# hilo-mpc/hilo-mpc

Hardware: AMD Instinct MI355X
Metric: MPC steps/sec (batched instances, whole node) at fixed (nx,nu,N) (higher is better)
Workload: dtype f64

## Files before the change

hilo_mpc_amd/csrc/hilo_nmpc_track.h:

```cpp
#pragma once
#include "hilo_ocp.h"

namespace hilo {

template <class M, bool BIG_ = false, bool SYM_ = true>
struct NmpcTrack {
  using Model = M;
  static constexpr bool SYM = SYM_ && ModelSym<M>::value && !model_has_ext<M>::value;
  static constexpr int NX = M::NX, NU = M::NU, NZ = NX + NU, NPAR = M::NP + M::NU, NSD = 0;
  static constexpr bool FIX_X0 = true;
  static constexpr bool BIG = BIG_;
  static constexpr int NC = 0, NXV = NX, NX0 = NX, NU0 = NU;
  static constexpr bool COOP = model_has_ext<M>::value;
  static constexpr bool QUAD_COST = true;
  static constexpr int O_WZ = 0, O_ZREF = O_WZ + NZ * NZ, O_WN = O_ZREF + NZ, O_XREFN = O_WN + NX * NX,
                       O_WDU = O_XREFN + NX, O_HASDU = O_WDU + NU * NU, O_SZ = O_HASDU + 1, O_SDU = O_SZ + NZ * NZ;
  static constexpr bool SYMTAB = O_SDU + NU * NU <= OCP_NCOST;
  static constexpr int O_END = SYMTAB ? O_SDU + NU * NU : O_SZ;
  static constexpr int NCOST = O_END;

  template <class T, class E>
  __device__ __forceinline__ static void dyn(const OcpConst& pc, const double* par, const double*, int, const T* x,
                                             const T* u, T* xn, const E& ext) {
    T xp[NX], up[NU > 0 ? NU : 1], xo[NX];
#pragma unroll
    for (int i = 0; i < NX; ++i) xp[i] = x[i] * pc.sz[i];
#pragma unroll
    for (int i = 0; i < NU; ++i) up[i] = u[i] * pc.sz[NX + i];
    model_step<M>(pc.order, pc.nsub, xp, up, par, pc.dt, xo, ext);
#pragma unroll
    for (int i = 0; i < NX; ++i) xn[i] = xo[i] * rcp_fast(pc.sz[i]);
  }

  static constexpr bool PLANT = !COOP;
  __device__ __forceinline__ static void plant(const OcpConst& pc, const double* par, const double* x, const double* u, double* xn) {
    if constexpr (PLANT) {
      double xv[NX], uv[NU > 0 ? NU : 1], pv[M::NP > 0 ? M::NP : 1], xo[NX];
#pragma unroll
      for (int i = 0; i < NX; ++i) xv[i] = x[i];
#pragma unroll
      for (int i = 0; i < NU; ++i) uv[i] = u[i];
#pragma unroll
      for (int i = 0; i < M::NP; ++i) pv[i] = par[i];
      model_step<M>(pc.order, pc.nsub, xv, uv, pv, pc.dt, xo);
#pragma unroll
      for (int i = 0; i < NX; ++i) xn[i] = xo[i];
    }
  }

  template <class T>
  __device__ __forceinline__ static T stage_cost(const OcpConst& pc, const double* par, const double*, int k,
                                                 const T* x, const T* u) {
    T z[NZ];
#pragma unroll
    for (int i = 0; i < NX; ++i) z[i] = x[i] - pc.cost[O_ZREF + i];
#pragma unroll
    for (int i = 0; i < NU; ++i) z[NX + i] = u[i] - pc.cost[O_ZREF + NX + i];
    T acc = T(0.0);
#pragma unroll
    for (int i0 = 0; i0 < NZ; i0 += 2) {
      double w[2][NZ];
#pragma unroll
      for (int a = 0; a < 2; ++a)
#pragma unroll
        for (int j = 0; j < NZ; ++j) w[a][j] = pc.cost[O_WZ + (i0 + a < NZ ? i0 + a : i0) * NZ + j];
      asm volatile("");
#pragma unroll
      for (int a = 0; a < 2; ++a) {
        if (i0 + a < NZ) {
          T s = T(0.0);
#pragma unroll
          for (int j = 0; j < NZ; ++j) s = s + w[a][j] * z[j];
          acc = acc + z[i0 + a] * s;
        }
      }
    }
    if (k == 0 && pc.cost[O_HASDU] != 0.0) {
      T d[NU > 0 ? NU : 1];
#pragma unroll
      for (int i = 0; i < NU; ++i) d[i] = u[i] - par[M::NP + i];
#pragma unroll
      for (int i = 0; i < NU; ++i) {
        T s = T(0.0);
#pragma unroll
        for (int j = 0; j < NU; ++j) s = s + pc.cost[O_WDU + i * NU + j] * d[j];
        acc = acc + d[i] * s;
      }
    }
    return acc;
  }

  __device__ __forceinline__ static double cost_grad(const OcpConst& pc, const double* par, const double*, int k, int i, const double* z) {
    double g = 0.0;
    {
      double wr[NZ], wc[NZ], zr[NZ];
#pragma unroll
      for (int j = 0; j < NZ; ++j) { wr[j] = pc.cost[O_WZ + i * NZ + j]; wc[j] = pc.cost[O_WZ + j * NZ + i]; zr[j] = pc.cost[O_ZREF + j]; }
      asm volatile("");
#pragma unroll
      for (int j = 0; j < NZ; ++j) g += (wr[j] + wc[j]) * (z[j] - zr[j]);
    }
    if (k == 0 && i >= NX && pc.cost[O_HASDU] != 0.0) {
#pragma unroll
      for (int j = 0; j < NU; ++j)
        g += (pc.cost[O_WDU + (i - NX) * NU + j] + pc.cost[O_WDU + j * NU + (i - NX)]) * (z[NX + j] - par[M::NP + j]);
    }
    return g;
  }
  __device__ __forceinline__ static double cost_hess(const OcpConst& pc, int k, int i, int j) {
    double h = pc.cost[O_WZ + i * NZ + j] + pc.cost[O_WZ + j * NZ + i];
    if (k == 0 && i >= NX && j >= NX && pc.cost[O_HASDU] != 0.0)
      h += pc.cost[O_WDU + (i - NX) * NU + (j - NX)] + pc.cost[O_WDU + (j - NX) * NU + (i - NX)];
    return h;
  }

  template <int CPL>
  __device__ __forceinline__ static void cost_cols(const OcpConst& pc, const double* par, int k, int c0, const double* z,
                                                   double* g, double (*ch)[CPL]) {
    static_assert(SYMTAB, "cost_cols needs the symmetrised tables");
    double S[NZ][CPL], zr[NZ], Sd[NU > 0 ? NU : 1][CPL], uo[NU > 0 ? NU : 1];
    int col[CPL], cu[CPL];
#pragma unroll
    for (int c = 0; c < CPL; ++c) {
      col[c] = c0 + c < NZ ? c0 + c : NZ - 1;
      cu[c] = col[c] >= NX ? col[c] - NX : 0;
    }
#pragma unroll
    for (int r = 0; r < NZ; ++r) {
      zr[r] = pc.cost[O_ZREF + r];
#pragma unroll
      for (int c = 0; c < CPL; ++c) S[r][c] = pc.cost[O_SZ + r * NZ + col[c]];
    }
#pragma unroll
    for (int a = 0; a < NU; ++a) {
      uo[a] = par[M::NP + a];
#pragma unroll
      for (int c = 0; c < CPL; ++c) Sd[a][c] = pc.cost[O_SDU + a * NU + cu[c]];
    }
    const bool du = k == 0 && pc.cost[O_HASDU] != 0.0;
#pragma unroll
    for (int c = 0; c < CPL; ++c) {
      double acc = 0.0;
#pragma unroll
      for (int r = 0; r < NZ; ++r) acc += S[r][c] * (z[r] - zr[r]);
      const bool duc = du && col[c] >= NX;
      double acd = acc;
#pragma unroll
      for (int a = 0; a < NU; ++a) acd += Sd[a][c] * (z[NX + a] - uo[a]);
      g[c] = duc ? acd : acc;
#pragma unroll
      for (int r = 0; r < NZ; ++r) {
        double h = S[r][c];
        if (r >= NX) h = duc ? h + Sd[r >= NX ? r - NX : 0][c] : h;
        ch[r][c] = (c0 + c < NZ && r >= c0 + c) ? h : 0.0;
      }
    }
  }

  __device__ __forceinline__ static double term_grad(const OcpConst& pc, int i, const double* x) {
    double g = 0.0;
#pragma unroll
    for (int j = 0; j < NX; ++j) g += (pc.cost[O_WN + i * NX + j] + pc.cost[O_WN + j * NX + i]) * (x[j] - pc.cost[O_XREFN + j]);
    return g;
  }
  __device__ __forceinline__ static double term_hess(const OcpConst& pc, int i, int j) {
    return pc.cost[O_WN + i * NX + j] + pc.cost[O_WN + j * NX + i];
  }

  template <class T>
  __device__ __forceinline__ static T term_cost(const OcpConst& pc, const double*, const double*, const T* x) {
    T z[NX];
#pragma unroll
    for (int i = 0; i < NX; ++i) z[i] = x[i] - pc.cost[O_XREFN + i];
    T acc = T(0.0);
// ... 24 lines not shown
```

hilo_mpc_amd/csrc/hilo_ocp.h:

```cpp
#pragma once
#include "hilo_colloc.h"
#include "hilo_common.h"
#include "hilo_models.h"

namespace hilo {

constexpr int OCP_MAXNX = 12, OCP_MAXNU = 8, OCP_MAXNZ = OCP_MAXNX + OCP_MAXNU;
constexpr int OCP_FILTER = 16;
constexpr int OCP_MAXNC = 16;
#ifndef HILO_OCP_TPB
#define HILO_OCP_TPB 64
#endif
#ifndef HILO_OCP_MINW
#define HILO_OCP_MINW 1
#endif
#ifdef HILO_OCP_INLINE_PHASES
#define OCP_PHASE __attribute__((always_inline))
#else
#define OCP_PHASE __attribute__((noinline))
#endif
constexpr int OCP_TPB = HILO_OCP_TPB;
constexpr int OCP_NCOST = 2 * OCP_MAXNZ * OCP_MAXNZ + 4 * OCP_MAXNZ + 64;

struct OcpConst {
// ... 379 lines not shown
    return (k > 0 && ((pc.k0_only_mask >> i) & 1u)) ? -INFINITY : pc.lbz[i];
  }
  __device__ static double ub_of(const OcpConst& pc, int k, int i) {
    if (k == 0 && (pc.flags & 2) && i < NX0) return pc.x0ub[i];
    return (k > 0 && ((pc.k0_only_mask >> i) & 1u)) ? INFINITY : pc.ubz[i];
  }

  __device__ __forceinline__ static void pair_of(int d, int n, int& i, int& j) {
    int r = d - n, ii = 0;
    for (int t = 0; t + 1 < n; ++t) {
      const int w = n - 1 - ii;
      const bool go = r >= w;
      r -= go ? w : 0;
      ii += go ? 1 : 0;
    }
    i = ii;
    j = ii + 1 + r;
  }
  __device__ static int dir_of(int i, int j, int n) { return n + i * (n - 1) - i * (i - 1) / 2 + (j - i - 1); }
  __device__ static bool pair_on(const OcpConst& pc, int d) {
    const int p = d - NZ;
    return p >= 256 || ((pc.pair_mask[p >> 6] >> (p & 63)) & 1ull) != 0ull;
  }
  __device__ static void build_dirs(const Lds l) {
    const OcpConst& pc = *(const OcpConst*)l.pc;
    if (threadIdx.x == 0) {
      int n = 0;
      for (int d = 0; d < NDIR; ++d)
        if (d < NZ || pair_on(pc, d)) l.dirs[1 + n++] = d;
      l.dirs[0] = n;
    }
    __syncthreads();
  }

  __device__ static const double* sd_of(const Lds l, int k) { return (const double*)(l.sd + (NSD > 0 ? k * NSD : 0)); }

  __device__ OCP_PHASE static FTheta eval_values_call(lds_double* lbase, double* ws, cvp Zp, ep cp, cdp sp, dp dstore, double extra) {
    lbase = uni(lbase); ws = uni(ws); Zp = uni(Zp); cp = uni(cp); sp = uni(sp); dstore = uni(dstore);
    const Lds l = carve(lbase, ws);
    const OcpConst& pc = *(const OcpConst*)l.pc;
    const int N = pc.N;
    double fpart = 0.0, tpart = 0.0;
    if constexpr (COOP) {
      const int lane = threadIdx.x;
      int gs = 64 / N;
      gs = gs < 1 ? 1 : gs;
      const int ng = 64 / gs, g = lane / gs, gl = lane - g * gs;
      const double* gp = (const double*)pc.ext;
      for (int r = 0; r * ng < N; ++r) {
        const int k = r * ng + g;
        const bool active = g < ng && k < N;
        const int kk = active ? k : N - 1;
        int nev = 0;
        const GpExt ext{gp, l.ext, gs, active ? gl : 0, active ? g * gs : lane, !active, (lds_cdouble*)(l.ext + NEXT_SCR),
                        pc.nsub == 1 ? l.gpc + kk * 24 : nullptr, &nev, false};
        double x[NX], u[NU > 0 ? NU : 1], xn[NX];
#pragma unroll
        for (int i = 0; i < NX; ++i) x[i] = Zp[kk * NZ + i];
#pragma unroll
        for (int i = 0; i < NU; ++i) u[i] = Zp[kk * NZ + NX + i];
        PB::dyn(pc, (const double*)l.par, sd_of(l, kk), kk, x, u, xn, ext);
        if (active && gl == 0) {
          fpart += PB::stage_cost(pc, (const double*)l.par, sd_of(l, k), k, x, u);
#pragma unroll
          for (int i = 0; i < NX; ++i) {
            const double ci = Zp[(k + 1) * NZ + i] - xn[i];
            cp[k * NX + i] = ci;
            tpart += fabs(ci);
          }
        }
      }
      if (lane == 63) {
        double x[NX];
#pragma unroll
        for (int i = 0; i < NX; ++i) x[i] = Zp[N * NZ + i];
        fpart += PB::term_cost(pc, (const double*)l.par, sd_of(l, N), x);
      }
    } else {
    if constexpr (XCW > 0) PB::template coll_pass<false>(pc, (const double*)l.par, (const double*)l.sd, Zp, l.lam, l.cnu, N, l.xc, l.prep, l.prepl,
                                                         uni((size_t)Zp != (size_t)l.Z));
#ifdef HILO_DBG_TWICE_VALS
    if constexpr (XCW > 0) PB::template coll_pass<false>(pc, (const double*)l.par, (const double*)l.sd, Zp, l.lam, l.cnu, N, l.xc, l.prep, l.prepl);
#endif
    OCP_FOR(k, (N) + 1) {
      double x[NX], u[NU > 0 ? NU : 1];
#pragma unroll
      for (int i = 0; i < NX; ++i) x[i] = Zp[k * NZ + i];
      if (k < N) {
        double xn[NX];
#pragma unroll
        for (int i = 0; i < NU; ++i) u[i] = Zp[k * NZ + NX + i];
        double dvf[NC > 0 ? NC : 1];
        if constexpr (XCW > 0) {
          fpart += PB::dyn_cost_xc(pc, (const double*)l.par, sd_of(l, k), k, x, u, xn, dvf, l.xc + (size_t)k * XCW);
        } else if constexpr (FUSED_CON) {
          static_assert(!FUSED_CON || FUSED, "fused rows need the fused cost");
          fpart += PB::dyn_cost_con(pc, (const double*)l.par, sd_of(l, k), k, x, u, xn, dvf, NoExt{});
        } else if constexpr (FUSED) {
          fpart += PB::dyn_cost(pc, (const double*)l.par, sd_of(l, k), k, x, u, xn, NoExt{});
        } else if constexpr (SYM) {
          using M = typename PB::Model;
          double xp[NX], up[NU > 0 ? NU : 1], X[4][NX], phi[NX];
#pragma unroll
          for (int i = 0; i < NX; ++i) xp[i] = x[i] * pc.sz[i];
#pragma unroll
          for (int i = 0; i < NU; ++i) up[i] = u[i] * pc.sz[NX + i];
          sym_points<M>(M::DISCRETE ? 1 : pc.order, pc.dt, xp, up, (const double*)l.par, X, phi);
          dp xs = l.Xs + (size_t)k * 4 * NX;
#pragma unroll
          for (int i = 0; i < 4; ++i)
#pragma unroll
            for (int q = 0; q < NX; ++q) xs[i * NX + q] = X[i][q];
#pragma unroll
          for (int i = 0; i < NX; ++i) xn[i] = phi[i] * rcp_fast(pc.sz[i]);
          fpart += PB::stage_cost(pc, (const double*)l.par, sd_of(l, k), k, x, u);
        } else {
          if constexpr (SYM_MHE) {
            FastD xf[NX], uf[NU > 0 ? NU : 1], xnf[NX];
#pragma unroll
            for (int i = 0; i < NX; ++i) xf[i] = FastD(x[i]);
#pragma unroll
            for (int i = 0; i < NU; ++i) uf[i] = FastD(u[i]);
            PB::dyn(pc, (const double*)l.par, sd_of(l, k), k, xf, uf, xnf, NoExt{});
#pragma unroll
            for (int i = 0; i < NX; ++i) xn[i] = xnf[i].v;
          } else {
            PB::dyn(pc, (const double*)l.par, sd_of(l, k), k, x, u, xn, NoExt{});
          }
          fpart += PB::stage_cost(pc, (const double*)l.par, sd_of(l, k), k, x, u);
        }
#pragma unroll
        for (int i = 0; i < NX; ++i) {
          const double ci = Zp[(k + 1) * NZ + i] - xn[i];
          cp[k * NX + i] = ci;
          tpart += fabs(ci);
        }
        if constexpr (NC > 0) {
          double dv[NC];
          if constexpr (FUSED_CON) {
#pragma unroll
            for (int m = 0; m < NC; ++m) dv[m] = dvf[m];
          } else PB::con(pc, (const double*)l.par, sd_of(l, k), k, x, u, xn, dv);
#pragma unroll
          for (int m = 0; m < NC; ++m) {
            if (row_on(pc, k, m)) {
              if (dstore) dstore[k * NC + m] = dv[m];
              if (sp) tpart += fabs(dv[m] - sp[k * NC + m]);
            }
          }
        }
      } else {
        fpart += PB::term_cost(pc, (const double*)l.par, sd_of(l, N), x);
      }
    }
    }
    if constexpr (OCP_TPB == 64) {
      double rv[3] = {fpart, tpart, extra};
      WaveReduceN<R_SUM, R_SUM, R_SUM>::run(rv);
      return FTheta{rv[0], rv[1], rv[2]};
    } else {
      const double fr = block_reduce<OpSum>(fpart, l.red);
      const double tr = block_reduce<OpSum>(tpart, l.red);
      return FTheta{fr, tr, block_reduce<OpSum>(extra, l.red)};
    }
  }

  __device__ __forceinline__ static FTheta eval_values(lds_double* lbase, double* ws, cvp Zp, ep cp, cdp sp = nullptr,
                                                      dp dstore = nullptr, double extra = 0.0) {
    const FTheta r = eval_values_call(lbase, ws, Zp, cp, sp, dstore, extra);
    return FTheta{uni(r.f), uni(r.theta), uni(r.x)};
  }

  template <bool TRIAL>
  __device__ __forceinline__ static double slots_log(const Lds l, cvp Zp, double alpha, int N) {
    constexpr int U = 2;
    const int SLT = (N + 1) * NZ;
    double part = 0.0;
    for (int base = 0; base < SLT; base += OCP_TPB * U) {
      double lbv[U], ubv[U], zv[U], dv[U];
      bool ok[U];
#pragma unroll
      for (int u = 0; u < U; ++u) {
        const int e0 = base + u * OCP_TPB + (int)threadIdx.x;
        ok[u] = e0 < SLT;
        const int e = ok[u] ? e0 : 0;
        lbv[u] = l.lbA[e]; ubv[u] = l.ubA[e]; zv[u] = Zp[e];
        dv[u] = TRIAL ? l.D[e] : 0.0;
      }
      double prod = 1.0;
      bool pos = true;
#pragma unroll
      for (int u = 0; u < U; ++u) {
        const double z = TRIAL ? zv[u] + alpha * dv[u] : zv[u];
        if constexpr (TRIAL) {
          if (ok[u]) l.Zt[base + u * OCP_TPB + (int)threadIdx.x] = z;
        }
        const bool hl = ok[u] && lbv[u] > -INFINITY, hu = ok[u] && ubv[u] < INFINITY;
        const double sl = hl ? z - lbv[u] : 1.0, su = hu ? ubv[u] - z : 1.0;
        prod *= sl * su;
        pos = pos && sl > 0.0 && su > 0.0;
      }
      const double r = -log(prod);
      part += pos ? r : __builtin_nan("");
    }
    return part;
  }
  __device__ static double barrier_logs(const Lds l, cvp Zp, cdp sp = nullptr) {
    const OcpConst& pc = *(const OcpConst*)l.pc;
    const int N = pc.N;
    double part = slots_log<false>(l, Zp, 0.0, N);
    if constexpr (NC > 0) {
      OCP_FOR(e, N * NC) {
        const int m = e % NC;
        if (!row_on(pc, e / NC, m)) continue;
        if (pc.dlb[m] > -INFINITY) part -= log(sp[e] - pc.dlb[m]);
        if (pc.dub[m] < INFINITY) part -= log(pc.dub[m] - sp[e]);
// ... 196 lines not shown
        if (d >= NX) pair_of(d, NX, di, dj);
        Jet2 x[NX];
#pragma unroll
        for (int i = 0; i < NX; ++i) x[i] = Jet2(l.Z[N * NZ + i], (i == di || i == dj) ? 1.0 : 0.0, 0.0);
        const Jet2 v = PB::term_cost(pc, (const double*)l.par, sd_of(l, N), x);
        qd_term(l, N)[d] = v.b;
        if (d < NX) l.grad[N * NZ + d] = v.a;
        if (d == 0) l.fk[N] = v.v;
      }
      }
    }
#ifdef HILO_DBG_TWICE_DIRS
    }
#endif
    __syncthreads();
    if constexpr (BIG) {
      constexpr int U = 4;
      const int total = N * NZ * NZ;
      for (int base = 0; base < total; base += OCP_TPB * U) {
        double qd[U], qa[U], qb[U];
        int kk[U], ii[U], jj[U];
        bool on[U], ok[U];
#pragma unroll
        for (int u = 0; u < U; ++u) {
          const int e0 = base + u * OCP_TPB + (int)threadIdx.x;
          ok[u] = e0 < total;
          const int e = ok[u] ? e0 : 0;
          const int k = e / (NZ * NZ), r = e - k * NZ * NZ, i = r / NZ, j = r - i * NZ;
          const int a = i < j ? i : j, b = i < j ? j : i;
          const int dd = i == j ? i : dir_of(a, b, NZ);
          cdp Q = l.Qd + k * NDIR;
          qd[u] = Q[dd]; qa[u] = Q[a]; qb[u] = Q[b];
          kk[u] = k; ii[u] = i; jj[u] = j;
          on[u] = i == j || COOP || pair_on(pc, dd);
        }
#pragma unroll
        for (int u = 0; u < U; ++u) {
          const int k = kk[u], i = ii[u], j = jj[u];
          double h = i == j ? qd[u] : (on[u] ? 0.5 * (qd[u] - qa[u] - qb[u]) : 0.0);
          if constexpr (PB::QUAD_COST) h += PB::cost_hess(pc, k, i, j);
          if (k == 0 && (((pinm >> i) | (pinm >> j)) & 1u)) h = 0.0;
          if (ok[u]) l.W[(k * NZ + i) * WP + j] = h;
        }
      }
    } else {
      OCP_FOR(e, N * NZ * NZ) {
        const int k = e / (NZ * NZ), r = e - k * NZ * NZ, i = r / NZ, j = r - i * NZ;
        cdp Q = l.Qd + k * NDIR;
        double h;
        if (i == j) h = Q[i];
        else {
          const int a = i < j ? i : j, b = i < j ? j : i, dd = dir_of(a, b, NZ);
          h = (COOP || pair_on(pc, dd)) ? 0.5 * (Q[dd] - Q[a] - Q[b]) : 0.0;
        }
        if constexpr (PB::QUAD_COST) h += PB::cost_hess(pc, k, i, j);
        if (k == 0 && (((pinm >> i) | (pinm >> j)) & 1u)) h = 0.0;
        l.W[(k * NZ + i) * WP + j] = h;
      }
    }
    if constexpr (PB::QUAD_COST) {
      OCP_FOR(e, N * NZ) {
        const int k = e / NZ, i = e - k * NZ;
        if (is_free(pc, k, i)) l.grad[e] = PB::cost_grad(pc, (const double*)l.par, sd_of(l, k), k, i, (const double*)(l.Z + k * NZ));
      }
      OCP_FOR(k, N) {
        double x[NX], u[NU > 0 ? NU : 1];
#pragma unroll
        for (int i = 0; i < NX; ++i) x[i] = l.Z[k * NZ + i];
#pragma unroll
        for (int i = 0; i < NU; ++i) u[i] = l.Z[k * NZ + NX + i];
        l.fk[k] = PB::stage_cost(pc, (const double*)l.par, sd_of(l, k), k, x, u);
      }
      __syncthreads();
    }
    double fpart = 0.0;
    OCP_FOR(k, (N) + 1) fpart += l.fk[k];
    OCP_FOR(a, NU) l.grad[N * NZ + NX + a] = 0.0;
    const double f = block_reduce<OpSum>(fpart, l.red);
    __syncthreads();
    return f;
  }


  template <class M>
  __device__ __forceinline__ static void sym_points(int order, double h, const double* x, const double* u, const double* par,
                                                    double (*X)[NX], double* phi) {
    constexpr bool DISC = M::DISCRETE;
    const double a10 = order >= 2 ? 0.5 : 0.0, a20 = order == 3 ? -1.0 : 0.0, a21 = order == 3 ? 2.0 : (order == 4 ? 0.5 : 0.0),
                 a32 = order == 4 ? 1.0 : 0.0;
    const double hb[4] = {DISC ? 1.0 : h * erk_b<0>(order), DISC ? 0.0 : h * erk_b<1>(order), DISC ? 0.0 : h * erk_b<2>(order),
                          DISC ? 0.0 : h * erk_b<3>(order)};
    FastD kk[4][NX], uf[NU > 0 ? NU : 1];
#pragma unroll
    for (int i = 0; i < NU; ++i) uf[i] = FastD(u[i]);
#pragma unroll
    for (int i = 0; i < 4; ++i) {
      FastD Xf[NX];
#pragma unroll
      for (int s = 0; s < NX; ++s) {
        double acc = x[s];
        if (i == 1) acc += (h * a10) * kk[0][s].v;
        if (i == 2) acc += (h * a20) * kk[0][s].v + (h * a21) * kk[1][s].v;
        if (i == 3) acc += (h * a32) * kk[2][s].v;
        X[i][s] = acc;
        Xf[s] = FastD(acc);
      }
      if (i < order) {
        M::ode(Xf, uf, par, h, kk[i]);
      } else {
#pragma unroll
        for (int s = 0; s < NX; ++s) kk[i][s] = FastD(0.0);
      }
    }
#pragma unroll
    for (int s = 0; s < NX; ++s)
      phi[s] = (DISC ? 0.0 : x[s]) + hb[0] * kk[0][s].v + hb[1] * kk[1][s].v + hb[2] * kk[2][s].v + hb[3] * kk[3][s].v;
  }

  __device__ static void term_hess_dirs(const Lds l) {
    const OcpConst& pc = *(const OcpConst*)l.pc;
    const int N = pc.N;
    OCP_FOR(d, NXDIR) {
      int di = d, dj = -1;
      if (d >= NX) pair_of(d, NX, di, dj);
      double q = PB::term_hess(pc, di, di);
      if (dj >= 0) q += PB::term_hess(pc, dj, dj) + 2.0 * PB::term_hess(pc, di, dj);
      qd_term(l, N)[d] = q;
    }
  }

  __device__ __attribute__((always_inline)) static double eval_derivs_sym(lds_double* lbase, double* ws, bool reuse = false) {
    using M = typename PB::Model;
    using MS = ModelSym<M>;
    using SM = sym_masks<MS>;
    static_assert(PB::QUAD_COST && NC == 0 && !COOP && !FUSED && M::NX == NX && M::NU == NU, "SYM: plain tracking policies");
    constexpr bool DISC = M::DISCRETE;
    constexpr int CPL = 2, LPI = (NZ + CPL - 1) / CPL;
    const Lds l = carve(lbase, ws);
    const OcpConst& pc = *(const OcpConst*)l.pc;
    const int N = pc.N;
    const int order = DISC ? 1 : pc.order;
    const double h = pc.dt;
    const unsigned pinm = FIX_X0 ? (~pc.x0_free_mask) & ((1u << NX) - 1u) : 0u;
    const double a10 = order >= 2 ? 0.5 : 0.0, a20 = order == 3 ? -1.0 : 0.0, a21 = order == 3 ? 2.0 : (order == 4 ? 0.5 : 0.0),
                 a32 = order == 4 ? 1.0 : 0.0;
    const double hb[4] = {DISC ? 1.0 : h * erk_b<0>(order), DISC ? 0.0 : h * erk_b<1>(order), DISC ? 0.0 : h * erk_b<2>(order),
                          DISC ? 0.0 : h * erk_b<3>(order)};
    const double* par = (const double*)l.par;
    DTICK0
    double fpart = 0.0;
    OCP_FOR(a, NU) l.grad[N * NZ + NX + a] = 0.0;
    DTICK(7)
    constexpr int IPP = OCP_TPB / LPI;
    static_assert(IPP >= 1, "SYM: more column groups than lanes");
    for (int kbase = 0; kbase < N; kbase += IPP) {
      const int li = (int)threadIdx.x / LPI;
      const bool act = li < IPP && kbase + li < N;
      const int k = act ? kbase + li : N - 1, g = act ? (int)threadIdx.x - li * LPI : 0, c0 = g * CPL;
      double zs[NZ], sz[NZ], isz[NX], x[NX], u[NU > 0 ? NU : 1], lamp[NX], X[4][NX], kb[4][NX];
#pragma unroll
      for (int i = 0; i < NZ; ++i) {
        zs[i] = l.Z[k * NZ + i];
        sz[i] = pc.sz[i];
      }
#pragma unroll
      for (int i = 0; i < NX; ++i) {
        isz[i] = rcp_fast(sz[i]);
        x[i] = zs[i] * sz[i];
        lamp[i] = l.lam[k * NX + i] * isz[i];
      }
#pragma unroll
      for (int i = 0; i < NU; ++i) u[i] = zs[NX + i] * sz[NX + i];
      DTICK(4)
      double ch[NZ][CPL];
      {
        double xN[NX];
#pragma unroll
        for (int i = 0; i < NX; ++i) xN[i] = l.Z[N * NZ + i];
        if constexpr (pb_symtab<PB>::value) {
          double gc[CPL];
          PB::template cost_cols<CPL>(pc, par, k, c0, zs, gc, ch);
          if (act) {
            if (g == 0 && !reuse) fpart += PB::stage_cost(pc, par, sd_of(l, k), k, zs, zs + NX);
            if (g == 0 && k == N - 1 && !reuse) fpart += PB::term_cost(pc, par, sd_of(l, N), xN);
#pragma unroll
            for (int c = 0; c < CPL; ++c) {
              const int col = c0 + c;
              if (col < NZ) l.grad[k * NZ + col] = is_free(pc, k, col) ? gc[c] : 0.0;
              if (col < NX && k == N - 1) l.grad[N * NZ + col] = PB::term_grad(pc, col, xN);
            }
          }
        } else {
        if (act) {
          if (g == 0 && !reuse) fpart += PB::stage_cost(pc, par, sd_of(l, k), k, zs, zs + NX);
          if (g == 0 && k == N - 1 && !reuse) fpart += PB::term_cost(pc, par, sd_of(l, N), xN);
#pragma unroll
          for (int c = 0; c < CPL; ++c) {
            const int col = c0 + c;
            if (col < NZ) l.grad[k * NZ + col] = is_free(pc, k, col) ? PB::cost_grad(pc, par, sd_of(l, k), k, col, zs) : 0.0;
            if (col < NX && k == N - 1) l.grad[N * NZ + col] = PB::term_grad(pc, col, xN);
          }
        }
#pragma unroll
        for (int c = 0; c < CPL; ++c)
#pragma unroll
          for (int r = 0; r < NZ; ++r) ch[r][c] = (c0 + c < NZ && r >= c0 + c) ? PB::cost_hess(pc, k, r, c0 + c) : 0.0;
        }
      }
      DTICK(5)
      if (!reuse) {
        double phi[NX];
        sym_points<M>(order, h, x, u, par, X, phi);
        if (act && g == 0) {
#pragma unroll
          for (int s = 0; s < NX; ++s) l.c[k * NX + s] = l.Z[(k + 1) * NZ + s] - phi[s] * isz[s];
        }
      } else {
        cdp xs = l.Xs + (size_t)k * 4 * NX;
#pragma unroll
        for (int i = 0; i < 4; ++i)
#pragma unroll
          for (int s = 0; s < NX; ++s) X[i][s] = xs[i * NX + s];
      }
      DTICK(0)
#pragma unroll
      for (int i = 0; i < 4; ++i)
#pragma unroll
        for (int s = 0; s < NX; ++s) kb[i][s] = hb[i] * lamp[s];
#pragma unroll
      for (int j = 3; j >= 1; --j) {
        if (j < order) {
          double fx[NX * NX], t[NX];
          MS::jx(X[j], u, par, fx);
#pragma unroll
          for (int n = 0; n < NX; ++n) {
            double acc = 0.0;
#pragma unroll
            for (int m = 0; m < NX; ++m)
              if ((SM::X >> (m * NX + n)) & 1ull) acc += fx[m * NX + n] * kb[j][m];
            t[n] = acc;
          }
#pragma unroll
          for (int n = 0; n < NX; ++n) {
            if (j == 3) kb[2][n] += (h * a32) * t[n];
            if (j == 2) { kb[1][n] += (h * a21) * t[n]; kb[0][n] += (h * a20) * t[n]; }
            if (j == 1) kb[0][n] += (h * a10) * t[n];
          }
        }
      }
      DTICK(1)
      dp scr = l.W + (size_t)k * NZ * WP;
      double dXc[NX][CPL], dX2[NX][CPL], dPhi[NX][CPL], G[NZ][CPL];
      double eU[NU > 0 ? NU : 1][CPL];
#pragma unroll
      for (int a = 0; a < NU; ++a)
#pragma unroll
        for (int c = 0; c < CPL; ++c) eU[a][c] = (c0 + c == NX + a) ? 1.0 : 0.0;
#pragma unroll
      for (int s = 0; s < NX; ++s)
#pragma unroll
        for (int c = 0; c < CPL; ++c) {
          dXc[s][c] = (c0 + c == s) ? 1.0 : 0.0;
          dX2[s][c] = dXc[s][c];
          dPhi[s][c] = DISC ? 0.0 : dXc[s][c];
        }
#pragma unroll
      for (int r = 0; r < NZ; ++r)
#pragma unroll
        for (int c = 0; c < CPL; ++c) G[r][c] = 0.0;
#pragma unroll
      for (int i = 0; i < 4; ++i) {
        if (i < order) {
          if (act) {
#pragma unroll
            for (int s = 0; s < NX; ++s)
#pragma unroll
              for (int c = 0; c < CPL; ++c)
                if (c0 + c < NZ) scr[s * NZ + c0 + c] = dXc[s][c];
          }
          __syncthreads();
          double dK[NX][CPL], v[NZ][CPL];
          {
            double J[NX * NZ], H[NZ * (NZ + 1) / 2];
            MS::jh(X[i], u, par, kb[i], J, H);
#pragma unroll
            for (int c = 0; c < CPL; ++c) {
#pragma unroll
              for (int m = 0; m < NX; ++m) {
                double acc = 0.0;
#pragma unroll
                for (int n = 0; n < NZ; ++n)
                  if ((SM::J >> (m * NZ + n)) & 1ull) acc += J[m * NZ + n] * (n < NX ? dXc[n < NX ? n : 0][c] : eU[n >= NX ? n - NX : 0][c]);
                dK[m][c] = acc;
              }
#pragma unroll
              for (int a = 0; a < NZ; ++a) {
                double acc = 0.0;
#pragma unroll
                for (int n = 0; n < NZ; ++n) {
                  const int q = a >= n ? a * (a + 1) / 2 + n : n * (n + 1) / 2 + a;
                  if ((SM::H >> q) & 1ull) acc += H[q] * (n < NX ? dXc[n < NX ? n : 0][c] : eU[n >= NX ? n - NX : 0][c]);
                }
                v[a][c] = acc;
              }
            }
          }
#pragma unroll
          for (int r = 0; r < NZ; ++r) {
            double col_r[NX];
#pragma unroll
            for (int a = 0; a < NX; ++a) col_r[a] = scr[a * NZ + r];
#pragma unroll
            for (int c = 0; c < CPL; ++c) {
              double acc = r >= NX ? v[r][c] : 0.0;
#pragma unroll
              for (int a = 0; a < NX; ++a) acc += col_r[a] * v[a][c];
              G[r][c] += acc;
            }
          }
#pragma unroll
          for (int s = 0; s < NX; ++s)
#pragma unroll
            for (int c = 0; c < CPL; ++c) {
              const double e = (c0 + c == s) ? 1.0 : 0.0;
              dPhi[s][c] += hb[i] * dK[s][c];
              if (i == 0) { dXc[s][c] = e + (h * a10) * dK[s][c]; dX2[s][c] = e + (h * a20) * dK[s][c]; }
              if (i == 1) dXc[s][c] = dX2[s][c] + (h * a21) * dK[s][c];
              if (i == 2) dXc[s][c] = e + (h * a32) * dK[s][c];
            }
          __syncthreads();
        }
      }
      DTICK(2)
      if (act) {
#pragma unroll
        for (int c = 0; c < CPL; ++c) {
          const int col = c0 + c;
          if (col < NZ) {
            const bool pin_c = k == 0 && ((pinm >> col) & 1u);
            double sc = sz[0];
#pragma unroll
            for (int r = 1; r < NZ; ++r) sc = col == r ? sz[r] : sc;
#pragma unroll
            for (int m = 0; m < NX; ++m) l.AB[(k * NX + m) * ABP + col] = pin_c ? 0.0 : dPhi[m][c] * sc * isz[m];
#pragma unroll
            for (int r = 0; r < NZ; ++r) {
              if (r >= col) {
                const bool pin = pin_c || (k == 0 && ((pinm >> r) & 1u));
                const double hv = pin ? 0.0 : ch[r][c] - sz[r] * sc * G[r][c];
                l.W[((size_t)k * NZ + r) * WP + col] = hv;
                l.W[((size_t)k * NZ + col) * WP + r] = hv;
              }
            }
          }
        }
      }
      DTICK(3)
    }
    __syncthreads();
    const double f = block_reduce<OpSum>(fpart, l.red);
    __syncthreads();
    DTICK(6)
    return f;
  }

  __device__ __attribute__((always_inline)) static double eval_derivs_sym_mhe(lds_double* lbase, double* ws) {
    using M = typename PB::Model;
    using MS = ModelSym<M>;
    constexpr int MU = PB::MU, NY = PB::NY, MZ = NX + MU, MU1 = MU > 0 ? MU : 1, NP = M::NP;
    static_assert(NU == NX && NC == 0 && !COOP && !FIX_X0 && NH == 0 && !M::DISCRETE && NX % 2 == 0, "SYM_MHE: the MheNoise policy");
    constexpr int CPL = 2, LPI = NX / CPL;
    const Lds l = carve(lbase, ws);
    const OcpConst& pc = *(const OcpConst*)l.pc;
    const int N = pc.N, order = pc.order;
    const double h = pc.dt;
    const double a10 = order >= 2 ? 0.5 : 0.0, a20 = order == 3 ? -1.0 : 0.0, a21 = order == 3 ? 2.0 : (order == 4 ? 0.5 : 0.0),
                 a32 = order == 4 ? 1.0 : 0.0;
    const double hb[4] = {h * erk_b<0>(order), h * erk_b<1>(order), h * erk_b<2>(order), h * erk_b<3>(order)};
    const double* par = (const double*)l.par;
    double fpart = 0.0;
    OCP_FOR(d, NXDIR) qd_term(l, N)[d] = 0.0;
    OCP_FOR(a, NZ) l.grad[N * NZ + a] = 0.0;
    constexpr int IPP = OCP_TPB / LPI;
    for (int kbase = 0; kbase < N; kbase += IPP) {
      const int li = (int)threadIdx.x / LPI;
      const bool act = li < IPP && kbase + li < N;
      const int k = act ? kbase + li : N - 1, g = act ? (int)threadIdx.x - li * LPI : 0, c0 = g * CPL;
      const double* sd = sd_of(l, k);
      double xsv[NX], wv[NX], sz[NX], sw[NX], isz[NX], x[NX], ue[MU1], lamp[NX], X[4][NX], kb[4][NX];
#pragma unroll
      for (int i = 0; i < NX; ++i) {
        xsv[i] = l.Z[k * NZ + i];
        wv[i] = l.Z[k * NZ + NX + i];
        sz[i] = pc.sz[i];
        sw[i] = pc.sz[NX + i];
        isz[i] = rcp_fast(sz[i]);
        x[i] = xsv[i] * sz[i];
        lamp[i] = l.lam[k * NX + i] * isz[i];
      }
#pragma unroll
      for (int i = 0; i < MU; ++i) ue[i] = sd[i] * pc.cost[PB::O_SU + i];
      double chx[NX][CPL], chw[NX][CPL], gx[CPL], gw[CPL];
      {
        double Jy[NY * NX], Hy[NX * (NX + 1) / 2], kby[NY], r[NY], yv[NY], ws_[NX];
        double val = 0.0;
        if (k == 0) {
          double d[NX];
#pragma unroll
          for (int i = 0; i < NX; ++i) d[i] = x[i] - par[NP + i];
#pragma unroll
          for (int i = 0; i < NX; ++i)
#pragma unroll
            for (int j = 0; j < NX; ++j) val += d[i] * pc.cost[PB::O_WX + i * NX + j] * d[j];
// ... 2146 lines not shown
```

Measured before the change: 6.534 million.

## Hoist scaling/RK tables out of loops and skip identity first-stage Hessian product

Precomputes the uniform RK coefficient table, scaled parameters and state scalings once per kernel instead of per stage. Adds a request/compute split for stage cost so the weight loads are issued before the RK evaluation. In the Hessian directional sweep, the first RK stage, where the scratch matrix is the identity, now skips the shared-memory write, both barriers and the NX-contraction when the block has 64 threads. A NaN check triggers a full recompute on that path so NaN propagation stays the same, at the cost of some extra code and register pressure.

```diff
diff --git a/hilo_mpc_amd/csrc/hilo_nmpc_track.h b/hilo_mpc_amd/csrc/hilo_nmpc_track.h
--- a/hilo_mpc_amd/csrc/hilo_nmpc_track.h
+++ b/hilo_mpc_amd/csrc/hilo_nmpc_track.h
@@ -90,6 +90,47 @@
     return acc;
   }
 
+  struct StageW { double w[NZ][NZ], zr[NZ], hasdu; };
+  __device__ __forceinline__ static void stage_cost_request(const OcpConst& pc, StageW& q) {
+#pragma unroll
+    for (int i = 0; i < NZ; ++i) {
+      q.zr[i] = pc.cost[O_ZREF + i];
+#pragma unroll
+      for (int j = 0; j < NZ; ++j) q.w[i][j] = pc.cost[O_WZ + i * NZ + j];
+    }
+    q.hasdu = pc.cost[O_HASDU];
+    asm volatile("");
+  }
+  __device__ __forceinline__ static double stage_cost_requested(const OcpConst& pc, const double* par, int k, const double* x,
+                                                                const double* u, const StageW& q) {
+    double z[NZ];
+#pragma unroll
+    for (int i = 0; i < NX; ++i) z[i] = x[i] - q.zr[i];
+#pragma unroll
+    for (int i = 0; i < NU; ++i) z[NX + i] = u[i] - q.zr[NX + i];
+    double acc = 0.0;
+#pragma unroll
+    for (int i = 0; i < NZ; ++i) {
+      double s = 0.0;
+#pragma unroll
+      for (int j = 0; j < NZ; ++j) s = s + q.w[i][j] * z[j];
+      acc = acc + z[i] * s;
+    }
+    if (k == 0 && q.hasdu != 0.0) {
+      double d[NU > 0 ? NU : 1];
+#pragma unroll
+      for (int i = 0; i < NU; ++i) d[i] = u[i] - par[M::NP + i];
+#pragma unroll
+      for (int i = 0; i < NU; ++i) {
+        double s = 0.0;
+#pragma unroll
+        for (int j = 0; j < NU; ++j) s = s + pc.cost[O_WDU + i * NU + j] * d[j];
+        acc = acc + d[i] * s;
+      }
+    }
+    return acc;
+  }
+
   __device__ __forceinline__ static double cost_grad(const OcpConst& pc, const double* par, const double*, int k, int i, const double* z) {
     double g = 0.0;
     {
diff --git a/hilo_mpc_amd/csrc/hilo_ocp.h b/hilo_mpc_amd/csrc/hilo_ocp.h
--- a/hilo_mpc_amd/csrc/hilo_ocp.h
+++ b/hilo_mpc_amd/csrc/hilo_ocp.h
@@ -485,12 +485,26 @@
 #ifdef HILO_DBG_TWICE_VALS
     if constexpr (XCW > 0) PB::template coll_pass<false>(pc, (const double*)l.par, (const double*)l.sd, Zp, l.lam, l.cnu, N, l.xc, l.prep, l.prepl);
 #endif
+    double vpar[NPAR], vsz[NZ], visz[NX];
+    SymTab vtb = SymTab();
+    int vorder = 1;
+    double vh = 0.0;
+    if constexpr (SYM) {
+      sym_par(l.par, vpar);
+#pragma unroll
+      for (int i = 0; i < NZ; ++i) vsz[i] = pc.sz[i];
+#pragma unroll
+      for (int i = 0; i < NX; ++i) visz[i] = rcp_fast(vsz[i]);
+      vorder = PB::Model::DISCRETE ? 1 : uni(pc.order);
+      vh = uni(pc.dt);
+      vtb = sym_tab<PB::Model::DISCRETE>(vorder, vh);
+    }
     OCP_FOR(k, (N) + 1) {
       double x[NX], u[NU > 0 ? NU : 1];
 #pragma unroll
       for (int i = 0; i < NX; ++i) x[i] = Zp[k * NZ + i];
       if (k < N) {
-        double xn[NX];
+        double xn[NX], zn[NX];
 #pragma unroll
         for (int i = 0; i < NU; ++i) u[i] = Zp[k * NZ + NX + i];
         double dvf[NC > 0 ? NC : 1];
@@ -505,18 +519,23 @@
           using M = typename PB::Model;
           double xp[NX], up[NU > 0 ? NU : 1], X[4][NX], phi[NX];
 #pragma unroll
-          for (int i = 0; i < NX; ++i) xp[i] = x[i] * pc.sz[i];
-#pragma unroll
-          for (int i = 0; i < NU; ++i) up[i] = u[i] * pc.sz[NX + i];
-          sym_points<M>(M::DISCRETE ? 1 : pc.order, pc.dt, xp, up, (const double*)l.par, X, phi);
+          for (int i = 0; i < NX; ++i) zn[i] = Zp[(k + 1) * NZ + i];
+          typename PB::StageW sw;
+          PB::stage_cost_request(pc, sw);
+          const double lk = PB::stage_cost_requested(pc, vpar, k, x, u, sw);
+#pragma unroll
+          for (int i = 0; i < NX; ++i) xp[i] = x[i] * vsz[i];
+#pragma unroll
+          for (int i = 0; i < NU; ++i) up[i] = u[i] * vsz[NX + i];
+          sym_points<M>(vorder, vh, vtb, xp, up, vpar, X, phi);
           dp xs = l.Xs + (size_t)k * 4 * NX;
 #pragma unroll
           for (int i = 0; i < 4; ++i)
 #pragma unroll
             for (int q = 0; q < NX; ++q) xs[i * NX + q] = X[i][q];
 #pragma unroll
-          for (int i = 0; i < NX; ++i) xn[i] = phi[i] * rcp_fast(pc.sz[i]);
-          fpart += PB::stage_cost(pc, (const double*)l.par, sd_of(l, k), k, x, u);
+          for (int i = 0; i < NX; ++i) xn[i] = phi[i] * visz[i];
+          fpart += lk;
         } else {
           if constexpr (SYM_MHE) {
             FastD xf[NX], uf[NU > 0 ? NU : 1], xnf[NX];
@@ -534,7 +553,10 @@
         }
 #pragma unroll
         for (int i = 0; i < NX; ++i) {
-          const double ci = Zp[(k + 1) * NZ + i] - xn[i];
+          double zi;
+          if constexpr (SYM) zi = zn[i];
+          else zi = Zp[(k + 1) * NZ + i];
+          const double ci = zi - xn[i];
           cp[k * NX + i] = ci;
           tpart += fabs(ci);
         }
@@ -897,14 +919,25 @@
   }
 
 
-  template <class M>
-  __device__ __forceinline__ static void sym_points(int order, double h, const double* x, const double* u, const double* par,
-                                                    double (*X)[NX], double* phi) {
-    constexpr bool DISC = M::DISCRETE;
+  struct SymTab { double ha10, ha20, ha21, ha32, hb[4]; };
+  template <bool DISC>
+  __device__ __forceinline__ static SymTab sym_tab(int order, double h) {
     const double a10 = order >= 2 ? 0.5 : 0.0, a20 = order == 3 ? -1.0 : 0.0, a21 = order == 3 ? 2.0 : (order == 4 ? 0.5 : 0.0),
                  a32 = order == 4 ? 1.0 : 0.0;
-    const double hb[4] = {DISC ? 1.0 : h * erk_b<0>(order), DISC ? 0.0 : h * erk_b<1>(order), DISC ? 0.0 : h * erk_b<2>(order),
-                          DISC ? 0.0 : h * erk_b<3>(order)};
+    return SymTab{uni(h * a10), uni(h * a20), uni(h * a21), uni(h * a32),
+                  {uni(DISC ? 1.0 : h * erk_b<0>(order)), uni(DISC ? 0.0 : h * erk_b<1>(order)), uni(DISC ? 0.0 : h * erk_b<2>(order)),
+                   uni(DISC ? 0.0 : h * erk_b<3>(order))}};
+  }
+  template <class LP>
+  __device__ __forceinline__ static void sym_par(LP lpar, double* parv) {
+#pragma unroll
+    for (int i = 0; i < NPAR; ++i) parv[i] = i < PB::NPAR ? uni(lpar[i < PB::NPAR ? i : 0]) : 0.0;
+  }
+
+  template <class M>
+  __device__ __forceinline__ static void sym_points(int order, double h, const SymTab& tb, const double* x, const double* u,
+                                                    const double* par, double (*X)[NX], double* phi) {
+    constexpr bool DISC = M::DISCRETE;
     FastD kk[4][NX], uf[NU > 0 ? NU : 1];
 #pragma unroll
     for (int i = 0; i < NU; ++i) uf[i] = FastD(u[i]);
@@ -914,9 +947,9 @@
 #pragma unroll
       for (int s = 0; s < NX; ++s) {
         double acc = x[s];
-        if (i == 1) acc += (h * a10) * kk[0][s].v;
-        if (i == 2) acc += (h * a20) * kk[0][s].v + (h * a21) * kk[1][s].v;
-        if (i == 3) acc += (h * a32) * kk[2][s].v;
+        if (i == 1) acc += tb.ha10 * kk[0][s].v;
+        if (i == 2) acc += tb.ha20 * kk[0][s].v + tb.ha21 * kk[1][s].v;
+        if (i == 3) acc += tb.ha32 * kk[2][s].v;
         X[i][s] = acc;
         Xf[s] = FastD(acc);
       }
@@ -929,7 +962,7 @@
     }
 #pragma unroll
     for (int s = 0; s < NX; ++s)
-      phi[s] = (DISC ? 0.0 : x[s]) + hb[0] * kk[0][s].v + hb[1] * kk[1][s].v + hb[2] * kk[2][s].v + hb[3] * kk[3][s].v;
+      phi[s] = (DISC ? 0.0 : x[s]) + tb.hb[0] * kk[0][s].v + tb.hb[1] * kk[1][s].v + tb.hb[2] * kk[2][s].v + tb.hb[3] * kk[3][s].v;
   }
 
   __device__ static void term_hess_dirs(const Lds l) {
@@ -954,15 +987,18 @@
     const Lds l = carve(lbase, ws);
     const OcpConst& pc = *(const OcpConst*)l.pc;
     const int N = pc.N;
-    const int order = DISC ? 1 : pc.order;
-    const double h = pc.dt;
+    const int order = DISC ? 1 : uni(pc.order);
+    const double h = uni(pc.dt);
     const unsigned pinm = FIX_X0 ? (~pc.x0_free_mask) & ((1u << NX) - 1u) : 0u;
-    const double a10 = order >= 2 ? 0.5 : 0.0, a20 = order == 3 ? -1.0 : 0.0, a21 = order == 3 ? 2.0 : (order == 4 ? 0.5 : 0.0),
-                 a32 = order == 4 ? 1.0 : 0.0;
-    const double hb[4] = {DISC ? 1.0 : h * erk_b<0>(order), DISC ? 0.0 : h * erk_b<1>(order), DISC ? 0.0 : h * erk_b<2>(order),
-                          DISC ? 0.0 : h * erk_b<3>(order)};
-    const double* par = (const double*)l.par;
     DTICK0
+    const SymTab tb = sym_tab<DISC>(order, h);
+    double parv[NPAR], sz[NZ], isz[NX];
+    sym_par(l.par, parv);
+    const double* par = parv;
+#pragma unroll
+    for (int i = 0; i < NZ; ++i) sz[i] = uni(pc.sz[i]);
+#pragma unroll
+    for (int i = 0; i < NX; ++i) isz[i] = uni(rcp_fast(sz[i]));
     double fpart = 0.0;
     OCP_FOR(a, NU) l.grad[N * NZ + NX + a] = 0.0;
     DTICK(7)
@@ -972,15 +1008,11 @@
       const int li = (int)threadIdx.x / LPI;
       const bool act = li < IPP && kbase + li < N;
       const int k = act ? kbase + li : N - 1, g = act ? (int)threadIdx.x - li * LPI : 0, c0 = g * CPL;
-      double zs[NZ], sz[NZ], isz[NX], x[NX], u[NU > 0 ? NU : 1], lamp[NX], X[4][NX], kb[4][NX];
-#pragma unroll
-      for (int i = 0; i < NZ; ++i) {
-        zs[i] = l.Z[k * NZ + i];
-        sz[i] = pc.sz[i];
-      }
+      double zs[NZ], x[NX], u[NU > 0 ? NU : 1], lamp[NX], X[4][NX], kb[4][NX];
+#pragma unroll
+      for (int i = 0; i < NZ; ++i) zs[i] = l.Z[k * NZ + i];
 #pragma unroll
       for (int i = 0; i < NX; ++i) {
-        isz[i] = rcp_fast(sz[i]);
         x[i] = zs[i] * sz[i];
         lamp[i] = l.lam[k * NX + i] * isz[i];
       }
@@ -1025,7 +1057,7 @@
       DTICK(5)
       if (!reuse) {
         double phi[NX];
-        sym_points<M>(order, h, x, u, par, X, phi);
+        sym_points<M>(order, h, tb, x, u, par, X, phi);
         if (act && g == 0) {
 #pragma unroll
           for (int s = 0; s < NX; ++s) l.c[k * NX + s] = l.Z[(k + 1) * NZ + s] - phi[s] * isz[s];
@@ -1041,7 +1073,7 @@
 #pragma unroll
       for (int i = 0; i < 4; ++i)
 #pragma unroll
-        for (int s = 0; s < NX; ++s) kb[i][s] = hb[i] * lamp[s];
+        for (int s = 0; s < NX; ++s) kb[i][s] = tb.hb[i] * lamp[s];
 #pragma unroll
       for (int j = 3; j >= 1; --j) {
         if (j < order) {
@@ -1057,9 +1089,9 @@
           }
 #pragma unroll
           for (int n = 0; n < NX; ++n) {
-            if (j == 3) kb[2][n] += (h * a32) * t[n];
-            if (j == 2) { kb[1][n] += (h * a21) * t[n]; kb[0][n] += (h * a20) * t[n]; }
-            if (j == 1) kb[0][n] += (h * a10) * t[n];
+            if (j == 3) kb[2][n] += tb.ha32 * t[n];
+            if (j == 2) { kb[1][n] += tb.ha21 * t[n]; kb[0][n] += tb.ha20 * t[n]; }
+            if (j == 1) kb[0][n] += tb.ha10 * t[n];
           }
         }
       }
@@ -1086,14 +1118,18 @@
 #pragma unroll
       for (int i = 0; i < 4; ++i) {
         if (i < order) {
-          if (act) {
-#pragma unroll
-            for (int s = 0; s < NX; ++s)
-#pragma unroll
-              for (int c = 0; c < CPL; ++c)
-                if (c0 + c < NZ) scr[s * NZ + c0 + c] = dXc[s][c];
-          }
-          __syncthreads();
+          constexpr bool UNIT = OCP_TPB == 64;
+          const bool unit0 = UNIT && i == 0;
+          if (!unit0) {
+            if (act) {
+#pragma unroll
+              for (int s = 0; s < NX; ++s)
+#pragma unroll
+                for (int c = 0; c < CPL; ++c)
+                  if (c0 + c < NZ) scr[s * NZ + c0 + c] = dXc[s][c];
+            }
+            __syncthreads();
+          }
           double dK[NX][CPL], v[NZ][CPL];
           {
             double J[NX * NZ], H[NZ * (NZ + 1) / 2];
@@ -1120,30 +1156,70 @@
               }
             }
           }
-#pragma unroll
-          for (int r = 0; r < NZ; ++r) {
-            double col_r[NX];
-#pragma unroll
-            for (int a = 0; a < NX; ++a) col_r[a] = scr[a * NZ + r];
-#pragma unroll
-            for (int c = 0; c < CPL; ++c) {
-              double acc = r >= NX ? v[r][c] : 0.0;
-#pragma unroll
-              for (int a = 0; a < NX; ++a) acc += col_r[a] * v[a][c];
-              G[r][c] += acc;
+          bool redo = false;
+          if (unit0) {
+            double chk = 0.0;
+#pragma unroll
+            for (int a = 0; a < NX; ++a)
+#pragma unroll
+              for (int c = 0; c < CPL; ++c) chk += v[a][c] * 0.0;
+            redo = __any((int)(chk != chk)) != 0;
+          }
+          if (!unit0) {
+#pragma unroll
+            for (int r = 0; r < NZ; ++r) {
+              double col_r[NX];
+#pragma unroll
+              for (int a = 0; a < NX; ++a) col_r[a] = scr[a * NZ + r];
+#pragma unroll
+              for (int c = 0; c < CPL; ++c) {
+                double acc = r >= NX ? v[r][c] : 0.0;
+#pragma unroll
+                for (int a = 0; a < NX; ++a) acc += col_r[a] * v[a][c];
+                G[r][c] += acc;
+              }
             }
+          } else {
+#pragma unroll
+            for (int r = 0; r < NZ; ++r)
+#pragma unroll
+              for (int c = 0; c < CPL; ++c) G[r][c] = v[r][c];
           }
 #pragma unroll
           for (int s = 0; s < NX; ++s)
 #pragma unroll
             for (int c = 0; c < CPL; ++c) {
               const double e = (c0 + c == s) ? 1.0 : 0.0;
-              dPhi[s][c] += hb[i] * dK[s][c];
-              if (i == 0) { dXc[s][c] = e + (h * a10) * dK[s][c]; dX2[s][c] = e + (h * a20) * dK[s][c]; }
-              if (i == 1) dXc[s][c] = dX2[s][c] + (h * a21) * dK[s][c];
-              if (i == 2) dXc[s][c] = e + (h * a32) * dK[s][c];
+              dPhi[s][c] += tb.hb[i] * dK[s][c];
+              if (i == 0) { dXc[s][c] = e + tb.ha10 * dK[s][c]; dX2[s][c] = e + tb.ha20 * dK[s][c]; }
+              if (i == 1) dXc[s][c] = dX2[s][c] + tb.ha21 * dK[s][c];
+              if (i == 2) dXc[s][c] = e + tb.ha32 * dK[s][c];
             }
-          __syncthreads();
+          if (!unit0) __syncthreads();
+          if (redo) {
+            if (act) {
+#pragma unroll
+              for (int s = 0; s < NX; ++s)
+#pragma unroll
+                for (int c = 0; c < CPL; ++c)
+                  if (c0 + c < NZ) scr[s * NZ + c0 + c] = (c0 + c == s) ? 1.0 : 0.0;
+            }
+            __syncthreads();
+#pragma unroll
+            for (int r = 0; r < NZ; ++r) {
+              double col_r[NX];
+#pragma unroll
+              for (int a = 0; a < NX; ++a) col_r[a] = scr[a * NZ + r];
+#pragma unroll
+              for (int c = 0; c < CPL; ++c) {
+                double acc = r >= NX ? v[r][c] : 0.0;
+#pragma unroll
+                for (int a = 0; a < NX; ++a) acc += col_r[a] * v[a][c];
+                G[r][c] = 0.0 + acc;
+              }
+            }
+            __syncthreads();
+          }
         }
       }
       DTICK(2)
```

New measurement: 6.801 million, median of 6. +4.1%, better.
